# POSTECH-CVLab/NeRF-Downstream

Hardware: AMD Instinct MI355X
Metric: voxels/sec fwd+bwd Mink-ResNet14 on CO3D plenoxels (higher is better)
Workload: dtype f32

## Files before the change

### include/mink_hip.h

```cpp
#ifndef MINK_HIP_H
#define MINK_HIP_H

#include <stddef.h>
#include <stdint.h>

#ifdef __cplusplus
extern "C" {
#endif

#define MINK_OK 0
#define MINK_EINVAL (-1)
#define MINK_ELAUNCH (-2)

#define MINK_STATUS_RANGE 1u
#define MINK_STATUS_UNSORTED 2u
#define MINK_STATUS_NOT_ASCENDING 4u

const char *mink_last_error(void);
int mink_abi_version(void);


int64_t mink_table_capacity(int64_t n);

int64_t mink_unique_workspace_bytes(int64_t n);
// ... 171 lines not shown
int mink_bn_stats_from_sums(const double *sums, const double *n_total, int32_t C, float eps, float momentum,
                            float *mean, float *invstd, float *running_mean, float *running_var,
                            void *stream);
int mink_bn_bwd_from_sums(const float *dy, const float *x, const float *y, int64_t n, int32_t C,
                          const double *sums, const double *n_total, const float *mean,
                          const float *invstd, const float *gamma, int32_t relu, float *dx,
                          float *dresidual, float *scratch2c, void *stream);

int mink_bn_relu_pool_fwd(const float *x, int32_t C, const float *mean, const float *invstd,
                          const float *gamma, const float *beta, const int32_t *nbr, int64_t n_out,
                          int32_t K, float *y, void *stream);
int mink_bn_relu_pool_bwd(const float *dy_pool, const float *x, int64_t n, int32_t C, const float *mean,
                          const float *invstd, const float *gamma, const float *beta,
                          const int32_t *in2out, float *dx, float *dgamma, float *dbeta,
                          void *workspace, int64_t workspace_bytes, void *stream);

int mink_pool_max_fwd(const float *x, int32_t C, const int32_t *nbr, int64_t n_out, int32_t K, float *y, int32_t *arg,
                      void *stream);
int mink_pool_max_bwd(const float *dy, const int32_t *arg, int32_t C, const int32_t *nbr_t, int64_t n_in, int32_t K,
                      float *dx, void *stream);

int mink_pool_local_fwd(const float *x, int32_t ldx, int32_t C, const int32_t *nbr, int64_t n_out, int32_t K, int32_t mode,
                        float *y, int32_t *cnt, void *stream);
int mink_pool_local_bwd(const float *dy, int32_t C, const int32_t *nbr_t, int64_t n_in, int32_t K, int32_t mode,
                        const int32_t *cnt, float *dx, void *stream);
int mink_pool_local_max_fwd(const float *x, int32_t ldx, int32_t C, const int32_t *nbr, int64_t n_out, int32_t K, float *y,
                            int32_t *arg, void *stream);
int mink_pool_local_max_bwd(const float *dy, const int32_t *arg, int32_t C, const int32_t *nbr_t, int64_t n_in, int32_t K,
                            float *dx, void *stream);
int64_t mink_global_pool_workspace_bytes(int64_t n, int32_t C, int32_t B);
// ... 136 lines not shown
  int64_t ws_bytes;
} MinkExec;

typedef struct {
  MinkConvLayer conv;
  MinkNormLayer norm;
  const int32_t *nbr_pool;
  const int32_t *in2out;
  int64_t n, n_pool;
  const float *x;
  float *y;
  float *out;
  const float *g_out;
  void *xb;
  int32_t xb_ready;
} MinkStem;

typedef struct {
  MinkConvLayer conv1, conv2, down;
  MinkNormLayer norm1, norm2, normd;
  int64_t n_in, n_out;
  const float *x;
  float *y1, *h1, *y2, *yd, *sd, *out;
  const float *g_out;
  float *g_x;
  float *g_tmp;
} MinkBasicBlock;

int64_t mink_block_workspace_bytes(int64_t n_in, int64_t n_out, int32_t cin, int32_t cout);
int64_t mink_block_grad_scratch_floats(int64_t n_in, int64_t n_out, int32_t cin, int32_t cout, int32_t has_down);
// ... 94 lines not shown
```

### nerf_downstream_amd/_lib.py

```python
import ctypes
import os
import subprocess

_HERE = os.path.dirname(os.path.abspath(__file__))
LIB_PATH = os.environ.get("MINK_HIP_LIB") or os.path.join(_HERE, "libmink_hip.so")
CSRC = os.path.join(_HERE, "csrc")

_i32, _i64, _f32, _p = ctypes.c_int32, ctypes.c_int64, ctypes.c_float, ctypes.c_void_p


class KernelMapDesc(ctypes.Structure):

    _fields_ = [("in_table_keys", _p), ("in_table_vals", _p), ("in_cap", _i64), ("out_coords", _p), ("n_out", _i64),
                ("n_in", _i64), ("nbr", _p), ("nbr_t", _p), ("K", _i32), ("offsets", _i32 * 81),
                ("in_coords", _p), ("in_ts", _i32), ("blk_build", _i32), ("blk_table", _p), ("blk_base", _p), ("blk_slot", _p),
                ("blk_rowids", _p), ("blk_counter", _p), ("blk_cap", _i64)]


class ConvLayer(ctypes.Structure):

    _fields_ = [("w", _p), ("dw", _p), ("nbr", _p), ("nbr_t", _p), ("perm", _p), ("n_perm", _i64), ("K", _i32), ("cin", _i32),
                ("cout", _i32), ("stride", _i32)]


class NormLayer(ctypes.Structure):

    _fields_ = [("gamma", _p), ("beta", _p), ("running_mean", _p), ("running_var", _p), ("dgamma", _p), ("dbeta", _p),
                ("mean", _p), ("invstd", _p), ("momentum", _f32), ("eps", _f32)]


class Exec(ctypes.Structure):

    _fields_ = [("compute", _p), ("branch", _p), ("wgrad", _p), ("ws_compute", _p), ("ws_branch", _p), ("ws_wgrad", _p),
                ("ws_bytes", _i64)]


class Stem(ctypes.Structure):

    _fields_ = [("conv", ConvLayer), ("norm", NormLayer), ("nbr_pool", _p), ("in2out", _p), ("n", _i64), ("n_pool", _i64),
                ("x", _p), ("y", _p), ("out", _p), ("g_out", _p), ("xb", _p), ("xb_ready", _i32)]


class BasicBlock(ctypes.Structure):

    _fields_ = [("conv1", ConvLayer), ("conv2", ConvLayer), ("down", ConvLayer), ("norm1", NormLayer), ("norm2", NormLayer),
                ("normd", NormLayer), ("n_in", _i64), ("n_out", _i64), ("x", _p), ("y1", _p), ("h1", _p), ("y2", _p),
                ("yd", _p), ("sd", _p), ("out", _p), ("g_out", _p), ("g_x", _p), ("g_tmp", _p)]


class LevelMaps(ctypes.Structure):

    _fields_ = [("n", _i64), ("nbr3", _p), ("down3", _p), ("down1", _p), ("down3_t", _p), ("perm", _p), ("n_perm", _i64)]


class Net(ctypes.Structure):
# ... 111 lines not shown
    "mink_bn_stats": (ctypes.c_int, [_p, _i64, _i32, _f32, _f32, _p, _p, _p, _p, _p, _i64, _p]),
    "mink_bn_apply": (ctypes.c_int, [_p, _i64, _i32, _p, _p, _p, _p, _p, _i32, _p, _p]),
    "mink_bn_fwd": (ctypes.c_int, [_p, _i64, _i32, _f32, _f32, _p, _p, _p, _i32, _p, _p, _p, _p, _p, _p, _i64, _p]),
    "mink_bn_bwd": (ctypes.c_int, [_p, _p, _p, _i64, _i32, _p, _p, _p, _i32, _p, _p, _p, _p, _p, _i64, _p]),
    "mink_in_workspace_bytes": (_i64, [_i64, _i32, _i32]),
    "mink_in_fwd": (ctypes.c_int, [_p, _i64, _i32, _p, _i32, _f32, _p, _p, _p, _i32, _p, _p, _p, _p, _i64, _p]),
    "mink_in_bwd": (ctypes.c_int, [_p, _p, _p, _i64, _i32, _p, _i32, _p, _p, _p, _i32, _p, _p, _p, _p, _p, _i64, _p]),
    "mink_ln_workspace_bytes": (_i64, [_i64, _i32]),
    "mink_ln_fwd": (ctypes.c_int, [_p, _i64, _i32, _f32, _p, _p, _p, _i32, _p, _p, _p, _p]),
    "mink_ln_bwd": (ctypes.c_int, [_p, _p, _p, _i64, _i32, _p, _p, _p, _i32, _p, _p, _p, _p, _p, _i64, _p]),
    "mink_bn_reduce": (ctypes.c_int, [_i32, _p, _p, _p, _i64, _i32, _p, _p, _p, _p, _i64, _p]),
    "mink_bn_stats_from_sums": (ctypes.c_int, [_p, _p, _i32, _f32, _f32, _p, _p, _p, _p, _p]),
    "mink_bn_bwd_from_sums": (ctypes.c_int, [_p, _p, _p, _i64, _i32, _p, _p, _p, _p, _p, _i32, _p, _p, _p, _p]),
    "mink_bn_relu_pool_fwd": (ctypes.c_int, [_p, _i32, _p, _p, _p, _p, _p, _i64, _i32, _p, _p]),
    "mink_bn_relu_pool_bwd": (ctypes.c_int, [_p, _p, _i64, _i32, _p, _p, _p, _p, _p, _p, _p, _p, _p, _i64, _p]),
    "mink_eltwise": (ctypes.c_int, [_p, _p, _i64, _i32, _p, _p]),
    "mink_sgd_step": (ctypes.c_int, [_p, _p, _p, _i64, _f32, _f32, _f32, _i32, _p]),
    "mink_activation": (ctypes.c_int, [_p, _p, _p, _i32, _i64, _i32, _f32, _p, _p]),
    "mink_block_workspace_bytes": (_i64, [_i64, _i64, _i32, _i32]),
    "mink_block_grad_scratch_floats": (_i64, [_i64, _i64, _i32, _i32, _i32]),
    "mink_class_partition_batch": (ctypes.c_int, [_i32, _p, _p]),
    "mink_rows_to_bf16": (ctypes.c_int, [_p, _i64, _i32, _i32, _p, _p]),
    "mink_stem_conv_bf16s_supported": (ctypes.c_int, [_i64, _i64, _i32, _i32, _i32]),
    "mink_stem_conv_bf16s_stats_rows": (_i32, []),
    "mink_stem_conv_bf16s": (ctypes.c_int, [_p, _i64, _p, _i32, _p, _i64, _i32, _p, _i32, _p, _i32, _p]),
    "mink_bn_relu_pool_fwd_b16": (ctypes.c_int, [_p, _i32, _p, _p, _p, _p, _p, _i64, _i32, _p, _p]),
    "mink_bn_relu_pool_bwd_b16": (ctypes.c_int, [_p, _p, _i64, _i32, _p, _p, _p, _p, _p, _p, _p, _p, _i64, _p]),
    "mink_conv_wgrad_bn_relu_pool_b16": (
        ctypes.c_int,
        [_p, _i64, _i32, _p, _i32, _p, _i64, _p, _p, _p, _p, _p, _p, _p, _p, _i64, _i32, _p, _p, _i64, _p],
# ... 49 lines not shown
        if not os.path.exists(LIB_PATH):
            raise MinkHipError(
                f"{LIB_PATH} not found: the HIP backend is mandatory (no CPU fallback). "
                "Build it with `python -c 'import __graft_entry__ as g; g.build()'` or `make -C nerf_downstream_amd/csrc`."
            )
        import torch

        L = ctypes.CDLL(LIB_PATH)
        for name, (res, args) in SIGNATURES.items():
            fn = getattr(L, name)
            fn.restype, fn.argtypes = res, args
        if os.environ.get("MINK_BN_FOLD"):
            L.mink_bn_set_fold(int(os.environ["MINK_BN_FOLD"]))
        if os.environ.get("MINK_BN_SMALL"):
            L.mink_bn_set_small(int(os.environ["MINK_BN_SMALL"]))
        if os.environ.get("MINK_CONV_PIPELINE"):
            L.mink_conv_set_pipeline(int(os.environ["MINK_CONV_PIPELINE"]))
        _lib = L
    return _lib


def check(rc):
    if rc != 0:
        raise MinkHipError(f"libmink_hip: {lib().mink_last_error().decode()} (code {rc})")
```

### nerf_downstream_amd/csrc/elementwise.hip

```cpp
#include <algorithm>

#include "common.h"

namespace mink {

constexpr int EB = 256;
static bool g_bn_small = true;
static bool g_bn_fold_force = false;
static int g_bn_fold = 0;
constexpr int kRedBlocks = 2048;

__device__ __forceinline__ float4 ld4(const float *p) { return *reinterpret_cast<const float4 *>(p); }
__device__ __forceinline__ void st4(float *p, float4 v) { *reinterpret_cast<float4 *>(p) = v; }
template <bool B16>
__device__ __forceinline__ float4 ldx4(const float *p, int64_t i) {
  if constexpr (!B16) return *reinterpret_cast<const float4 *>(p + i);
  const uint2 u = *reinterpret_cast<const uint2 *>(reinterpret_cast<const unsigned short *>(p) + i);
  return make_float4(__uint_as_float(u.x << 16), __uint_as_float(u.x & 0xFFFF0000u), __uint_as_float(u.y << 16),
                     __uint_as_float(u.y & 0xFFFF0000u));
}

__device__ __forceinline__ void bn_running_update(float *running_mean, float *running_var, int c, float momentum, float m, double var, int64_t n) {
#pragma clang fp contract(off)
  const double unbiased = n > 1 ? var * (double)n / (double)(n - 1) : var;
// ... 670 lines not shown
    }
  }
}

template <bool BWD>
__global__ __launch_bounds__(EB) void activation_kernel(const float *__restrict__ x, const float *__restrict__ gy,
                                                        const float *__restrict__ slope, int C, int64_t count, int kind,
                                                        float alpha, float *__restrict__ out) {
  for (int64_t i = (int64_t)blockIdx.x * EB + threadIdx.x; i < count; i += (int64_t)gridDim.x * EB) {
    const float a = slope ? slope[C > 1 ? (int)(i % C) : 0] : alpha;
    const float v = act_eval<BWD>(kind, x[i], a);
    out[i] = BWD ? gy[i] * v : v;
  }
}

template <bool B16>
__global__ __launch_bounds__(EB) void bn_relu_pool_fwd_kernel(const float *__restrict__ x, int C4,
                                                              const float *__restrict__ mean,
                                                              const float *__restrict__ invstd,
                                                              const float *__restrict__ gamma,
                                                              const float *__restrict__ beta,
                                                              const int *__restrict__ nbr, int64_t n_out, int K,
                                                              float *__restrict__ y) {
  const int64_t idx = (int64_t)blockIdx.x * EB + threadIdx.x;
  if (idx >= n_out * C4) return;
  const int64_t o = idx / C4;
  const int c = (int)(idx - o * C4) * 4;
  const float4 mu = ld4(mean + c), is = ld4(invstd + c), g = ld4(gamma + c), b = ld4(beta + c);
  const float4 sc = make_float4(is.x * g.x, is.y * g.y, is.z * g.z, is.w * g.w);
  const float4 sh = make_float4(b.x - mu.x * sc.x, b.y - mu.y * sc.y, b.z - mu.z * sc.z, b.w - mu.w * sc.w);
  float4 s = make_float4(0, 0, 0, 0);
  auto add = [&](const float4 &v) {
    s.x += fmaxf((v.x - mu.x) * is.x * g.x + b.x, 0.f), s.y += fmaxf((v.y - mu.y) * is.y * g.y + b.y, 0.f);
    s.z += fmaxf((v.z - mu.z) * is.z * g.z + b.z, 0.f), s.w += fmaxf((v.w - mu.w) * is.w * g.w + b.w, 0.f);
  };
  if (K == 8) {
    int ch[8];
#pragma unroll
    for (int k = 0; k < 8; ++k) ch[k] = nbr[o * 8 + k];
    float4 v[8];
#pragma unroll
    for (int k = 0; k < 8; ++k) v[k] = ldx4<B16>(x, (int64_t)max(ch[k], 0) * (4 * C4) + c);
#pragma unroll
    for (int k = 0; k < 8; ++k)
      if (ch[k] >= 0) add(v[k]);
  } else {
    for (int k = 0; k < K; ++k) {
      const int i = nbr[o * K + k];
      if (i >= 0) add(ldx4<B16>(x, (int64_t)i * (4 * C4) + c));
    }
  }
  (void)sh;
  st4(y + o * (int64_t)(4 * C4) + c, s);
}

__global__ __launch_bounds__(EB) void bn_relu_pool_bwd_kernel(const float *__restrict__ dyp,
                                                              const float *__restrict__ x,
                                                              const int *__restrict__ in2out, int64_t n, int C4,
                                                              float inv_n, const float *__restrict__ mean,
                                                              const float *__restrict__ invstd,
                                                              const float *__restrict__ gamma,
                                                              const float *__restrict__ beta,
                                                              const float *__restrict__ dgamma,
                                                              const float *__restrict__ dbeta,
                                                              float *__restrict__ dx) {
  for (int64_t i4 = (int64_t)blockIdx.x * EB + threadIdx.x; i4 < n * C4; i4 += (int64_t)gridDim.x * EB) {
    const int64_t row = i4 / C4;
    const int c = (int)(i4 - row * C4) * 4;
// ... 463 lines not shown
  REQ_C4(C, "bn_bwd_from_sums");
  MINK_REQUIRE(n >= 1 && dy && x && sums && n_total && mean && invstd && gamma && dx && scratch2c,
               "bn_bwd_from_sums: bad arguments");
  MINK_REQUIRE(!relu || y, "bn_bwd_from_sums: fused ReLU needs the forward output");
  hipStream_t st = (hipStream_t)stream;
  bn_bwd_sums_to_float_kernel<<<dim3((unsigned)cdiv(C, 64)), 64, 0, st>>>(sums, n_total, C, scratch2c, scratch2c + C);
  MINK_CHECK_LAUNCH();
  const int64_t n4 = n * (C >> 2);
  bn_bwd_apply_kernel<<<dim3(ew_grid(n4)), EB, 0, st>>>(dy, x, relu ? y : nullptr, n4, C >> 2, 1.f, mean, invstd, gamma,
                                                       scratch2c + C, scratch2c, dx, dresidual);
  MINK_CHECK_LAUNCH();
  return MINK_OK;
}

static int bn_relu_pool_fwd_impl(const float *x, bool b16, int32_t C, const float *mean, const float *invstd, const float *gamma,
                                 const float *beta, const int32_t *nbr, int64_t n_out, int32_t K, float *y, void *stream) {
  REQ_C4(C, "bn_relu_pool_fwd");
  MINK_REQUIRE(n_out >= 0 && K >= 1, "bn_relu_pool_fwd: bad shape");
  if (n_out == 0) return MINK_OK;
  MINK_REQUIRE(x && mean && invstd && gamma && beta && nbr && y, "bn_relu_pool_fwd: NULL pointer");
  REQ_A16(x, "bn_relu_pool_fwd");
  REQ_A16(y, "bn_relu_pool_fwd");
  const dim3 grid((unsigned)cdiv(n_out * (C >> 2), EB));
  if (b16) bn_relu_pool_fwd_kernel<true><<<grid, EB, 0, (hipStream_t)stream>>>(x, C >> 2, mean, invstd, gamma, beta, nbr, n_out, K, y);
  else bn_relu_pool_fwd_kernel<false><<<grid, EB, 0, (hipStream_t)stream>>>(x, C >> 2, mean, invstd, gamma, beta, nbr, n_out, K, y);
  MINK_CHECK_LAUNCH();
  return MINK_OK;
}

int mink_bn_relu_pool_fwd(const float *x, int32_t C, const float *mean, const float *invstd, const float *gamma,
                          const float *beta, const int32_t *nbr, int64_t n_out, int32_t K, float *y, void *stream) {
  return bn_relu_pool_fwd_impl(x, false, C, mean, invstd, gamma, beta, nbr, n_out, K, y, stream);
}

int mink_bn_relu_pool_fwd_b16(const void *xb, int32_t C, const float *mean, const float *invstd, const float *gamma,
                              const float *beta, const int32_t *nbr, int64_t n_out, int32_t K, float *y, void *stream) {
  return bn_relu_pool_fwd_impl((const float *)xb, true, C, mean, invstd, gamma, beta, nbr, n_out, K, y, stream);
}

static int bn_relu_pool_bwd_impl(const float *dy_pool, const float *x, bool b16, int64_t n, int32_t C, const float *mean,
// ... 191 lines not shown
```

### nerf_downstream_amd/csrc/trunk.hip

```cpp
#include <algorithm>
#include <vector>

#include "common.h"

namespace mink {
namespace {

struct Scratch {
  char *base;
  int64_t bytes, off = 0;
  Scratch(void *p, int64_t n) : base((char *)p), bytes(n) {}
  void *take(int64_t n) {
    n = align_up(n > 0 ? n : 1, 256);
    if (!base || off + n > bytes) return nullptr;
    void *p = base + off;
    off += n;
    return p;
  }
};

constexpr int kEvents = 8;
hipEvent_t g_ev[kEvents];
bool g_ev_ready = false;

// ... 190 lines not shown
    const int rows = mink_stem_conv_bf16s_stats_rows();
    double *partial = (double *)ws.take((int64_t)rows * 2 * c.cout * sizeof(double));
    MINK_REQUIRE(partial, "stem_forward: scratch too small");
    if (!s->xb_ready) TRY(mink_rows_to_bf16(s->x, s->n, c.cin, c.cin, s->xb, st));
    TRY(mink_stem_conv_bf16s(s->xb, s->n, c.w, c.cin, c.nbr, s->n, c.K, s->y, c.cout, partial, rows, st));
    TRY(mink_bn_stats_from_partials(partial, rows, s->n, c.cout, s->norm.eps, s->norm.running_mean ? s->norm.momentum : 0.f, s->norm.mean,
                                    s->norm.invstd, s->norm.running_mean, s->norm.running_var, st));
    return mink_bn_relu_pool_fwd_b16(s->y, c.cout, s->norm.mean, s->norm.invstd, s->norm.gamma, s->norm.beta, s->nbr_pool, s->n_pool, 8,
                                     s->out, st);
  }
  ConvOut co;
  TRY(conv_stats(s->conv, s->norm, s->x, s->n, s->n, s->y, ex->ws_compute, ex->ws_bytes, st, co));
  if (co.rows > 0)
    TRY(mink_bn_stats_from_partials(co.partial, co.rows, s->n, s->conv.cout, s->norm.eps, s->norm.running_mean ? s->norm.momentum : 0.f,
                                    s->norm.mean, s->norm.invstd, s->norm.running_mean, s->norm.running_var, st));
  return mink_bn_relu_pool_fwd(s->y, s->conv.cout, s->norm.mean, s->norm.invstd, s->norm.gamma, s->norm.beta, s->nbr_pool,
                               s->n_pool, 8, s->out, st);
}

int mink_stem_backward(const MinkStem *s, const MinkExec *ex) {
  MINK_REQUIRE(s && ex, "stem_backward: NULL descriptor");
  TRY(check_conv(s->conv, "stem_backward", true));
  TRY(check_norm(s->norm, "stem_backward", true));
  MINK_REQUIRE(s->x && s->y && s->g_out && s->in2out && s->n >= 1 && s->n_pool >= 1, "stem_backward: bad arguments");
  hipStream_t st = (hipStream_t)ex->compute;
  Scratch ws(ex->ws_compute, ex->ws_bytes);
  void *bn_ws = ws.take(mink_bn_workspace_bytes(s->n, s->conv.cout));
  const int64_t need = mink_conv_wgrad_workspace_bytes(s->n, s->conv.K, s->conv.cin, s->conv.cout);
  void *slabs = need > 0 ? ws.take(need) : nullptr;
  MINK_REQUIRE(bn_ws && (need == 0 || slabs), "stem_backward: scratch too small");
  if (s->xb) {
    TRY(mink_bn_relu_pool_bwd_b16(s->g_out, s->y, s->n, s->conv.cout, s->norm.mean, s->norm.invstd, s->norm.gamma, s->norm.beta, s->in2out,
                                  s->norm.dgamma, s->norm.dbeta, bn_ws, mink_bn_workspace_bytes(s->n, s->conv.cout), st));
    return mink_conv_wgrad_bn_relu_pool_b16(s->xb, s->n, s->conv.cin, s->y, s->conv.cout, s->g_out, s->n_pool, s->in2out, s->norm.mean,
                                            s->norm.invstd, s->norm.gamma, s->norm.beta, s->norm.dgamma, s->norm.dbeta, s->conv.nbr,
                                            s->n, s->conv.K, s->conv.dw, slabs, need, st);
  }
  TRY(mink_bn_relu_pool_bwd(s->g_out, s->y, s->n, s->conv.cout, s->norm.mean, s->norm.invstd, s->norm.gamma, s->norm.beta,
                            s->in2out, nullptr, s->norm.dgamma, s->norm.dbeta, bn_ws, mink_bn_workspace_bytes(s->n, s->conv.cout), st));
  return mink_conv_wgrad_bn_relu_pool(s->x, s->n, s->conv.cin, s->conv.cin, s->y, s->conv.cout, s->g_out, s->n_pool, s->in2out,
                                      s->norm.mean, s->norm.invstd, s->norm.gamma, s->norm.beta, s->norm.dgamma,
                                      s->norm.dbeta, s->conv.nbr, s->n, s->conv.K, s->conv.dw, slabs, need, st);
}

int mink_block_forward(const MinkBasicBlock *b, const MinkExec *ex) {
  MINK_REQUIRE(b && ex, "block_forward: NULL descriptor");
  TRY(check_conv(b->conv1, "block_forward conv1", false));
  TRY(check_conv(b->conv2, "block_forward conv2", false));
  TRY(check_norm(b->norm1, "block_forward norm1", false));
  TRY(check_norm(b->norm2, "block_forward norm2", false));
  const bool down = b->down.w != nullptr;
  const int C = b->conv1.cout;
  MINK_REQUIRE(b->x && b->y1 && b->h1 && b->y2 && b->out && b->n_in >= 1 && b->n_out >= 1 && b->conv2.cin == C &&
                   b->conv2.cout == C,
// ... 172 lines not shown
  b.norm1.mean = st, b.norm1.invstd = st + C, b.norm2.mean = st + 2 * C, b.norm2.invstd = st + 3 * C;
  b.normd.mean = st + 4 * C, b.normd.invstd = st + 5 * C;
  b.conv2.nbr = lo.nbr3, b.conv2.nbr_t = nullptr, b.conv2.perm = nullptr, b.conv2.n_perm = 0;
  if (b.conv1.stride == 2) {
    b.conv1.nbr = lo.down3, b.conv1.nbr_t = lo.down3_t, b.conv1.perm = lo.perm, b.conv1.n_perm = lo.perm ? lo.n_perm : 0;
    MINK_REQUIRE(sh.down && lo.down1, "net: a strided block needs its shortcut convolution and the k=1 table");
    b.down.nbr = lo.down1, b.down.nbr_t = nullptr, b.down.perm = nullptr, b.down.n_perm = 0;
  } else {
    MINK_REQUIRE(!sh.down, "net: a stride-1 block with a shortcut convolution is not sequenced here");
    b.conv1.nbr = lo.nbr3, b.conv1.nbr_t = nullptr, b.conv1.perm = nullptr, b.conv1.n_perm = 0;
  }
  MINK_REQUIRE(b.conv1.nbr && b.conv2.nbr, "net: missing neighbour table at level %d", sh.level_out);
  return MINK_OK;
}

}

extern "C" {

int mink_set_block_done_hook(MinkBlockDoneHook hook) {
  g_block_done_hook = hook;
  return MINK_OK;
}

int mink_set_stage_hook(MinkStageHook hook) {
  g_stage_hook = hook;
  return MINK_OK;
}

int mink_event_create(void **event_out) {
// ... 14 lines not shown
  MINK_HIP(hipStreamWaitEvent((hipStream_t)stream, (hipEvent_t)event, 0));
  return MINK_OK;
}

int mink_net_sizes(const MinkNet *net, const MinkLevelMaps *levels, int32_t n_levels, int64_t *act_floats, int64_t *grad_floats,
                   int64_t *ws_bytes) {
  MINK_REQUIRE(net && levels && n_levels >= 1 && net->n_blocks >= 1 && net->blocks, "net_sizes: bad arguments");
  int64_t act = 0, grad = 0, ws = 0;
  int level = 0;
  for (int i = 0; i < net->n_blocks; ++i) {
    BlockShape sh;
    TRY(block_shape(net, levels, n_levels, i, level, sh));
    act += sh.act + sh.stats, grad += sh.gtmp + sh.gx;
    ws = std::max(ws, mink_block_workspace_bytes(sh.n_in, sh.n_out, net->blocks[i].conv1.cin, net->blocks[i].conv1.cout));
  }
  if (act_floats) *act_floats = act;
  if (grad_floats) *grad_floats = grad;
  if (ws_bytes) *ws_bytes = ws;
  return MINK_OK;
}

int mink_net_forward(MinkNet *net, const MinkLevelMaps *levels, int32_t n_levels, float *arena, int64_t arena_floats,
                     const MinkExec *ex) {
  MINK_REQUIRE(net && levels && arena && ex && net->blocks && net->n_blocks >= 1, "net_forward: bad arguments");
  if (g_stage_hook) g_stage_hook(-1, 0);
  if (net->with_stem) TRY(mink_stem_forward(&net->stem, ex));
  MINK_REQUIRE(net->stem.out && net->stem.n_pool == levels[0].n, "net_forward: the stem output must be level 0 (%lld rows, %lld given)",
               (long long)net->stem.n_pool, (long long)levels[0].n);
  const float *x = net->stem.out;
  int level = 0;
  int64_t off = 0;
  for (int i = 0; i < net->n_blocks; ++i) {
    BlockShape sh;
    TRY(block_shape(net, levels, n_levels, i, level, sh));
    MINK_REQUIRE(off + sh.act + sh.stats <= arena_floats, "net_forward: activation arena of %lld floats is too small (mink_net_sizes)",
                 (long long)arena_floats);
    MinkBasicBlock &b = net->blocks[i];
    TRY(bind_block(b, sh, levels, arena + off, x));
    b.g_out = nullptr, b.g_x = nullptr, b.g_tmp = nullptr;
    if (g_stage_hook) g_stage_hook(i, 0);
    TRY(mink_block_forward(&b, ex));
// ... 7 lines not shown

int mink_net_backward(MinkNet *net, const MinkLevelMaps *levels, int32_t n_levels, float *arena, int64_t arena_floats,
                      const float *g_out, float *grad_arena, int64_t grad_floats, const MinkExec *ex, void *const *done_events) {
  MINK_REQUIRE(net && levels && arena && g_out && grad_arena && ex && net->blocks && net->n_blocks >= 1, "net_backward: bad arguments");
  TRY(ensure_events());
  std::vector<BlockShape> shapes(net->n_blocks);
  std::vector<int64_t> offs(net->n_blocks);
  int level = 0;
  int64_t off = 0, goff_total = 0;
  for (int i = 0; i < net->n_blocks; ++i) {
    TRY(block_shape(net, levels, n_levels, i, level, shapes[i]));
    offs[i] = off;
    off += shapes[i].act + shapes[i].stats;
    goff_total += shapes[i].gtmp + shapes[i].gx;
  }
  MINK_REQUIRE(off <= arena_floats && goff_total <= grad_floats, "net_backward: arena too small (mink_net_sizes)");
  hipStream_t st = (hipStream_t)ex->compute, wst = (hipStream_t)ex->wgrad;
  const float *g = g_out;
  int64_t goff = 0;
  PendingGrad pending;
  for (int i = net->n_blocks - 1; i >= 0; --i) {
    const BlockShape &sh = shapes[i];
    MinkBasicBlock &b = net->blocks[i];
    const float *x = i == 0 ? net->stem.out : arena + offs[i - 1] + 3 * shapes[i - 1].n_out * net->blocks[i - 1].conv1.cout;
    TRY(bind_block(b, sh, levels, arena + offs[i], x));
    b.g_out = g, b.g_tmp = grad_arena + goff, b.g_x = grad_arena + goff + sh.gtmp;
    if (g_stage_hook) g_stage_hook(i, 1);
    const bool may_defer = i > 0 && shapes[i - 1].level_out == sh.level_out && net->blocks[i - 1].conv1.cout == b.conv1.cin;
    PendingGrad next;
    TRY(block_backward_impl(&b, ex, &pending, may_defer ? &next : nullptr));
    pending = next;
    const bool want_event = done_events && done_events[i];
    if (want_event || g_block_done_hook) {
      if (wst != st) TRY(order_after(wst, st, 7));
      if ((hipStream_t)ex->branch != st && (hipStream_t)ex->branch != wst) TRY(order_after(wst, (hipStream_t)ex->branch, 4));
      if (want_event) MINK_HIP(hipEventRecord((hipEvent_t)done_events[i], wst));
      if (g_block_done_hook) g_block_done_hook(i);
    }
    g = b.g_x;
    goff += sh.gtmp + sh.gx;
  }
  if (g_stage_hook) g_stage_hook(-1, 1);
  if (net->with_stem) {
    net->stem.g_out = g;
    TRY(mink_stem_backward(&net->stem, ex));
  }
  net->g_stem_out = g;
  return MINK_OK;
}

}
```

### nerf_downstream_amd/minkowski/functional.py

```python
import ctypes
import os

import torch

from .._lib import check, lib


def _stream():
    return torch._C._cuda_getCurrentRawStream(torch.cuda.current_device())


def _f32c(t):
    assert t.is_cuda, "the HIP backend has no CPU path"
    return t.contiguous() if t.dtype == torch.float32 else t.float().contiguous()


def _ptr(t):
    return None if t is None else t.data_ptr()


def _bytes(nbytes, device):
    return torch.empty(max(int(nbytes), 256), dtype=torch.uint8, device=device)


# ... 761 lines not shown
        )
        dbeta, dgamma = sums[:C].float(), sums[C:].float()
        dist.all_reduce(sums, group=ctx.group)
        gx = torch.empty_like(x)
        gres = torch.empty_like(x) if ctx.has_res else None
        tmp = torch.empty(2 * C, dtype=torch.float32, device=dev)
        check(
            L.mink_bn_bwd_from_sums(
                gy.data_ptr(), x.data_ptr(), _ptr(y), n, C, sums.data_ptr(), n_total.data_ptr(), mean.data_ptr(),
                invstd.data_ptr(), gamma.data_ptr(), int(ctx.relu), gx.data_ptr(), _ptr(gres), tmp.data_ptr(), _stream(),
            )
        )
        return gx, dgamma, dbeta, None, None, None, None, gres, None, None


class BNReLUSumPoolFunction(torch.autograd.Function):

    @staticmethod
    def forward(ctx, x, gamma, beta, running_mean, running_var, training, momentum, eps, nbr, in2out, partial=None):
        L = lib()
        x = _f32c(x)
        n, C = x.shape
        dev = x.device
        if training:
            mean, invstd = _bn_statistics(L, x, n, C, eps, momentum, running_mean, running_var, partial)
        else:
            mean = running_mean.float()
            invstd = torch.rsqrt(running_var.float() + eps)
        n_out, K = nbr.shape
        y = torch.empty(n_out, C, dtype=torch.float32, device=dev)
        check(
            L.mink_bn_relu_pool_fwd(
                x.data_ptr(), C, mean.data_ptr(), invstd.data_ptr(), gamma.data_ptr(), beta.data_ptr(), nbr.data_ptr(),
                n_out, K, y.data_ptr(), _stream(),
            )
        )
        ctx.save_for_backward(x, mean, invstd, gamma, beta)
        ctx.in2out, ctx.training = in2out, training
        return y

    @staticmethod
    def backward(ctx, gy):
        if not ctx.training:
            raise NotImplementedError("fused bn+relu+pool backward needs batch statistics (training mode)")
        L = lib()
        x, mean, invstd, gamma, beta = ctx.saved_tensors
        gy = _f32c(gy)
        n, C = x.shape
        gx = torch.empty_like(x)
        dgamma = torch.empty(C, dtype=torch.float32, device=x.device)
        dbeta = torch.empty(C, dtype=torch.float32, device=x.device)
        ws = _scratch(L.mink_bn_workspace_bytes(n, C), x.device, "bn")
        check(
            L.mink_bn_relu_pool_bwd(
                gy.data_ptr(), x.data_ptr(), n, C, mean.data_ptr(), invstd.data_ptr(), gamma.data_ptr(), beta.data_ptr(),
                ctx.in2out.data_ptr(), gx.data_ptr(), dgamma.data_ptr(), dbeta.data_ptr(), ws.data_ptr(), ws.numel(), _stream(),
            )
        )
        return gx, dgamma, dbeta, None, None, None, None, None, None, None, None


class ConvBNReLUSumPoolFunction(torch.autograd.Function):

    @staticmethod
    def forward(ctx, x, kernel, gamma, beta, running_mean, running_var, momentum, eps, nbr, nbr_pool, in2out):
        L = lib()
        x, w = _f32c(x), _f32c(kernel)
        cin = x.shape[1]
        ctx.cin = cin
        if cin % 4:
            pad = 4 - cin % 4
            x = torch.nn.functional.pad(x, (0, pad))
            w = torch.nn.functional.pad(w, (0, 0, 0, pad))
        C = w.shape[-1]
        y, partial = gather_gemm(x, w, nbr, C, stats=True)
        n = y.shape[0]
        mean, invstd = _bn_statistics(L, y, n, C, eps, momentum, running_mean, running_var, partial)
        n_pool, K = nbr_pool.shape
        out = torch.empty(n_pool, C, dtype=torch.float32, device=x.device)
        check(
            L.mink_bn_relu_pool_fwd(
                y.data_ptr(), C, mean.data_ptr(), invstd.data_ptr(), gamma.data_ptr(), beta.data_ptr(), nbr_pool.data_ptr(),
                n_pool, K, out.data_ptr(), _stream(),
            )
        )
        ctx.save_for_backward(x, w, y, mean, invstd, gamma, beta)
        ctx.nbr, ctx.in2out = nbr, in2out
        ctx.kernel = kernel
        return out

    @staticmethod
    def backward(ctx, gy):
        L = lib()
        x, w, y, mean, invstd, gamma, beta = ctx.saved_tensors
        gy = _f32c(gy)
        n, C = y.shape
        dev = y.device
        need = ctx.needs_input_grad
        pv = _sink_views(gamma, beta) if need[2] and need[3] else None
        kv = _sink_views(ctx.kernel) if need[1] and w.shape[1] == ctx.cin else None
        if pv is not None:
            dgamma, dbeta = pv
        else:
            dgamma = torch.empty(C, dtype=torch.float32, device=dev)
            dbeta = torch.empty(C, dtype=torch.float32, device=dev)
        gw = kv[0] if kv is not None else None
        ws = _scratch(L.mink_bn_workspace_bytes(n, C), dev, "bn")
        check(
            L.mink_bn_relu_pool_bwd(
                gy.data_ptr(), y.data_ptr(), n, C, mean.data_ptr(), invstd.data_ptr(), gamma.data_ptr(), beta.data_ptr(),
                ctx.in2out.data_ptr(), None, dgamma.data_ptr(), dbeta.data_ptr(), ws.data_ptr(), ws.numel(), _stream(),
            )
        )
        nbr = ctx.nbr
        K = nbr.shape[1]
        if gw is None:
            gw = torch.empty(w.shape, dtype=torch.float32, device=dev)
        wws = _scratch(L.mink_conv_wgrad_workspace_bytes(n, K, x.shape[1], C), dev, "wgrad")
        note_table(nbr)
        check(
            L.mink_conv_wgrad_bn_relu_pool(
                x.data_ptr(), x.shape[0], x.stride(0), x.shape[1], y.data_ptr(), C, gy.data_ptr(), gy.shape[0],
                ctx.in2out.data_ptr(), mean.data_ptr(), invstd.data_ptr(), gamma.data_ptr(), beta.data_ptr(),
                dgamma.data_ptr(), dbeta.data_ptr(), nbr.data_ptr(), n, K, gw.data_ptr(), wws.data_ptr(), wws.numel(), _stream(),
            )
        )
        if _GRAD_SINK is not None and hasattr(_GRAD_SINK, "flush"):
            _GRAD_SINK.flush()
# ... 537 lines not shown
```

Before: 241.3 million.

## Compute stem BN-ReLU-pool gradient reductions from pooled-resolution byproducts

The forward BN+ReLU+sum-pool kernel now also records, per pooled row and channel, the count of children that passed ReLU (uint8) and the sum of their normalized values. The backward dgamma/dbeta reduction then reads these pooled-resolution tensors instead of re-reading the full-resolution pre-pool activations with in2out indirection. This shrinks the reduction's memory traffic by roughly the pooling factor, at the cost of extra forward writes and extra arena memory. It is on by default and also changes the Python autograd path.

```diff
diff --git a/include/mink_hip.h b/include/mink_hip.h
--- a/include/mink_hip.h
+++ b/include/mink_hip.h
@@ -209,6 +209,17 @@
                           const float *invstd, const float *gamma, const float *beta,
                           const int32_t *in2out, float *dx, float *dgamma, float *dbeta,
                           void *workspace, int64_t workspace_bytes, void *stream);
+int mink_bn_relu_pool_fwd_stats(const float *x, int32_t C, const float *mean, const float *invstd, const float *gamma,
+                                const float *beta, const int32_t *nbr, int64_t n_out, int32_t K, float *y, uint8_t *cnt,
+                                float *xs, void *stream);
+int mink_bn_relu_pool_bwd_pooled(const float *dy_pool, const uint8_t *cnt, const float *xs, int64_t n_pool, int32_t C,
+                                 const float *gamma, float *dgamma, float *dbeta, void *workspace, int64_t workspace_bytes,
+                                 void *stream);
+int mink_bn_relu_pool_bwd_dx(const float *dy_pool, const float *x, int64_t n, int32_t C, const float *mean, const float *invstd,
+                             const float *gamma, const float *beta, const int32_t *in2out, const float *dgamma,
+                             const float *dbeta, float *dx, void *stream);
+int32_t mink_stem_pooled_bwd(void);
+int mink_stem_set_pooled_bwd(int32_t on);
 
 int mink_pool_max_fwd(const float *x, int32_t C, const int32_t *nbr, int64_t n_out, int32_t K, float *y, int32_t *arg,
                       void *stream);
@@ -375,6 +386,8 @@
   const float *g_out;
   void *xb;
   int32_t xb_ready;
+  uint8_t *pool_cnt;
+  float *pool_xs;
 } MinkStem;
 
 typedef struct {
diff --git a/nerf_downstream_amd/_lib.py b/nerf_downstream_amd/_lib.py
--- a/nerf_downstream_amd/_lib.py
+++ b/nerf_downstream_amd/_lib.py
@@ -38,7 +38,7 @@
 class Stem(ctypes.Structure):
 
     _fields_ = [("conv", ConvLayer), ("norm", NormLayer), ("nbr_pool", _p), ("in2out", _p), ("n", _i64), ("n_pool", _i64),
-                ("x", _p), ("y", _p), ("out", _p), ("g_out", _p), ("xb", _p), ("xb_ready", _i32)]
+                ("x", _p), ("y", _p), ("out", _p), ("g_out", _p), ("xb", _p), ("xb_ready", _i32), ("pool_cnt", _p), ("pool_xs", _p)]
 
 
 class BasicBlock(ctypes.Structure):
@@ -180,6 +180,11 @@
     "mink_bn_bwd_from_sums": (ctypes.c_int, [_p, _p, _p, _i64, _i32, _p, _p, _p, _p, _p, _i32, _p, _p, _p, _p]),
     "mink_bn_relu_pool_fwd": (ctypes.c_int, [_p, _i32, _p, _p, _p, _p, _p, _i64, _i32, _p, _p]),
     "mink_bn_relu_pool_bwd": (ctypes.c_int, [_p, _p, _i64, _i32, _p, _p, _p, _p, _p, _p, _p, _p, _p, _i64, _p]),
+    "mink_bn_relu_pool_fwd_stats": (ctypes.c_int, [_p, _i32, _p, _p, _p, _p, _p, _i64, _i32, _p, _p, _p, _p]),
+    "mink_bn_relu_pool_bwd_pooled": (ctypes.c_int, [_p, _p, _p, _i64, _i32, _p, _p, _p, _p, _i64, _p]),
+    "mink_bn_relu_pool_bwd_dx": (ctypes.c_int, [_p, _p, _i64, _i32, _p, _p, _p, _p, _p, _p, _p, _p, _p]),
+    "mink_stem_pooled_bwd": (_i32, []),
+    "mink_stem_set_pooled_bwd": (ctypes.c_int, [_i32]),
     "mink_eltwise": (ctypes.c_int, [_p, _p, _i64, _i32, _p, _p]),
     "mink_sgd_step": (ctypes.c_int, [_p, _p, _p, _i64, _f32, _f32, _f32, _i32, _p]),
     "mink_activation": (ctypes.c_int, [_p, _p, _p, _i32, _i64, _i32, _f32, _p, _p]),
@@ -259,6 +264,8 @@
             L.mink_bn_set_fold(int(os.environ["MINK_BN_FOLD"]))
         if os.environ.get("MINK_BN_SMALL"):
             L.mink_bn_set_small(int(os.environ["MINK_BN_SMALL"]))
+        if os.environ.get("MINK_STEM_POOLED_BWD"):
+            L.mink_stem_set_pooled_bwd(int(os.environ["MINK_STEM_POOLED_BWD"]))
         if os.environ.get("MINK_CONV_PIPELINE"):
             L.mink_conv_set_pipeline(int(os.environ["MINK_CONV_PIPELINE"]))
         _lib = L
diff --git a/nerf_downstream_amd/csrc/elementwise.hip b/nerf_downstream_amd/csrc/elementwise.hip
--- a/nerf_downstream_amd/csrc/elementwise.hip
+++ b/nerf_downstream_amd/csrc/elementwise.hip
@@ -8,6 +8,7 @@
 static bool g_bn_small = true;
 static bool g_bn_fold_force = false;
 static int g_bn_fold = 0;
+static bool g_pool_bwd = true;
 constexpr int kRedBlocks = 2048;
 
 __device__ __forceinline__ float4 ld4(const float *p) { return *reinterpret_cast<const float4 *>(p); }
@@ -708,14 +709,15 @@
   }
 }
 
-template <bool B16>
+template <bool B16, bool PROD = false>
 __global__ __launch_bounds__(EB) void bn_relu_pool_fwd_kernel(const float *__restrict__ x, int C4,
                                                               const float *__restrict__ mean,
                                                               const float *__restrict__ invstd,
                                                               const float *__restrict__ gamma,
                                                               const float *__restrict__ beta,
                                                               const int *__restrict__ nbr, int64_t n_out, int K,
-                                                              float *__restrict__ y) {
+                                                              float *__restrict__ y, unsigned char *__restrict__ cnt = nullptr,
+                                                              float *__restrict__ xs = nullptr) {
   const int64_t idx = (int64_t)blockIdx.x * EB + threadIdx.x;
   if (idx >= n_out * C4) return;
   const int64_t o = idx / C4;
@@ -724,9 +726,19 @@
   const float4 sc = make_float4(is.x * g.x, is.y * g.y, is.z * g.z, is.w * g.w);
   const float4 sh = make_float4(b.x - mu.x * sc.x, b.y - mu.y * sc.y, b.z - mu.z * sc.z, b.w - mu.w * sc.w);
   float4 s = make_float4(0, 0, 0, 0);
+  float4 hs = make_float4(0, 0, 0, 0);
+  unsigned pass = 0;
   auto add = [&](const float4 &v) {
-    s.x += fmaxf((v.x - mu.x) * is.x * g.x + b.x, 0.f), s.y += fmaxf((v.y - mu.y) * is.y * g.y + b.y, 0.f);
-    s.z += fmaxf((v.z - mu.z) * is.z * g.z + b.z, 0.f), s.w += fmaxf((v.w - mu.w) * is.w * g.w + b.w, 0.f);
+    const float4 t = make_float4((v.x - mu.x) * is.x * g.x + b.x, (v.y - mu.y) * is.y * g.y + b.y, (v.z - mu.z) * is.z * g.z + b.z,
+                                 (v.w - mu.w) * is.w * g.w + b.w);
+    s.x += fmaxf(t.x, 0.f), s.y += fmaxf(t.y, 0.f);
+    s.z += fmaxf(t.z, 0.f), s.w += fmaxf(t.w, 0.f);
+    if constexpr (PROD) {
+      if (t.x > 0.f) hs.x += (v.x - mu.x) * is.x, pass += 1u;
+      if (t.y > 0.f) hs.y += (v.y - mu.y) * is.y, pass += 1u << 8;
+      if (t.z > 0.f) hs.z += (v.z - mu.z) * is.z, pass += 1u << 16;
+      if (t.w > 0.f) hs.w += (v.w - mu.w) * is.w, pass += 1u << 24;
+    }
   };
   if (K == 8) {
     int ch[8];
@@ -746,6 +758,55 @@
   }
   (void)sh;
   st4(y + o * (int64_t)(4 * C4) + c, s);
+  if constexpr (PROD) {
+    st4(xs + o * (int64_t)(4 * C4) + c, hs);
+    *reinterpret_cast<unsigned *>(cnt + o * (int64_t)(4 * C4) + c) = pass;
+  }
+}
+
+constexpr int kPoolRows = 8;
+constexpr int kPoolRedBlocks = 1024;
+__global__ __launch_bounds__(EB) void bn_relu_pool_bwd_pooled_kernel(const float *__restrict__ g, const unsigned char *__restrict__ cnt,
+                                                                     const float *__restrict__ xs, int64_t n, int C,
+                                                                     double *__restrict__ partial) {
+  extern __shared__ double s_red[];
+  const int tpr = C >> 2, rlanes = EB / tpr;
+  const int c4 = threadIdx.x % tpr, rl = threadIdx.x / tpr;
+  if (rl < rlanes) {
+    double a0 = 0, a1 = 0, a2 = 0, a3 = 0, b0 = 0, b1 = 0, b2 = 0, b3 = 0;
+    const int64_t stride = (int64_t)gridDim.x * rlanes;
+    for (int64_t row = (int64_t)blockIdx.x * rlanes + rl; row < n; row += kPoolRows * stride) {
+      float4 gs[kPoolRows], hs[kPoolRows];
+      unsigned cs[kPoolRows];
+#pragma unroll
+      for (int u = 0; u < kPoolRows; ++u) {
+        const int64_t r = row + u * stride < n ? row + u * stride : row;
+        const int64_t off = r * C + 4 * c4;
+        gs[u] = ld4(g + off), hs[u] = ld4(xs + off);
+        cs[u] = *reinterpret_cast<const unsigned *>(cnt + off);
+      }
+#pragma unroll
+      for (int u = 0; u < kPoolRows; ++u) {
+        if (row + u * stride < n) {
+          const float4 gv = gs[u], hv = hs[u];
+          const unsigned cv = cs[u];
+          a0 += (double)gv.x * (double)(cv & 255u), a1 += (double)gv.y * (double)((cv >> 8) & 255u);
+          a2 += (double)gv.z * (double)((cv >> 16) & 255u), a3 += (double)gv.w * (double)(cv >> 24);
+          b0 += (double)gv.x * (double)hv.x, b1 += (double)gv.y * (double)hv.y;
+          b2 += (double)gv.z * (double)hv.z, b3 += (double)gv.w * (double)hv.w;
+        }
+      }
+    }
+    double *d = s_red + ((int64_t)rl * 2) * C + 4 * c4;
+    d[0] = a0, d[1] = a1, d[2] = a2, d[3] = a3;
+    d[C + 0] = b0, d[C + 1] = b1, d[C + 2] = b2, d[C + 3] = b3;
+  }
+  __syncthreads();
+  for (int e = threadIdx.x; e < 2 * C; e += EB) {
+    double t = 0.0;
+    for (int r = 0; r < rlanes; ++r) t += s_red[(int64_t)r * 2 * C + e];
+    partial[(int64_t)blockIdx.x * 2 * C + e] = t;
+  }
 }
 
 __global__ __launch_bounds__(EB) void bn_relu_pool_bwd_kernel(const float *__restrict__ dyp,
@@ -1239,16 +1300,74 @@
 }
 
 static int bn_relu_pool_fwd_impl(const float *x, bool b16, int32_t C, const float *mean, const float *invstd, const float *gamma,
-                                 const float *beta, const int32_t *nbr, int64_t n_out, int32_t K, float *y, void *stream) {
+                                 const float *beta, const int32_t *nbr, int64_t n_out, int32_t K, float *y, void *stream,
+                                 uint8_t *cnt = nullptr, float *xs = nullptr) {
   REQ_C4(C, "bn_relu_pool_fwd");
   MINK_REQUIRE(n_out >= 0 && K >= 1, "bn_relu_pool_fwd: bad shape");
+  MINK_REQUIRE((cnt == nullptr) == (xs == nullptr), "bn_relu_pool_fwd_stats: cnt and xs come in pairs");
+  MINK_REQUIRE(!cnt || (K <= 255 && !b16), "bn_relu_pool_fwd_stats: at most 255 children per pooled row, fp32 storage");
   if (n_out == 0) return MINK_OK;
   MINK_REQUIRE(x && mean && invstd && gamma && beta && nbr && y, "bn_relu_pool_fwd: NULL pointer");
   REQ_A16(x, "bn_relu_pool_fwd");
   REQ_A16(y, "bn_relu_pool_fwd");
+  REQ_A16(cnt, "bn_relu_pool_fwd_stats");
+  REQ_A16(xs, "bn_relu_pool_fwd_stats");
   const dim3 grid((unsigned)cdiv(n_out * (C >> 2), EB));
-  if (b16) bn_relu_pool_fwd_kernel<true><<<grid, EB, 0, (hipStream_t)stream>>>(x, C >> 2, mean, invstd, gamma, beta, nbr, n_out, K, y);
+  if (cnt) bn_relu_pool_fwd_kernel<false, true><<<grid, EB, 0, (hipStream_t)stream>>>(x, C >> 2, mean, invstd, gamma, beta, nbr, n_out, K, y, cnt, xs);
+  else if (b16) bn_relu_pool_fwd_kernel<true><<<grid, EB, 0, (hipStream_t)stream>>>(x, C >> 2, mean, invstd, gamma, beta, nbr, n_out, K, y);
   else bn_relu_pool_fwd_kernel<false><<<grid, EB, 0, (hipStream_t)stream>>>(x, C >> 2, mean, invstd, gamma, beta, nbr, n_out, K, y);
+  MINK_CHECK_LAUNCH();
+  return MINK_OK;
+}
+
+int mink_bn_relu_pool_fwd_stats(const float *x, int32_t C, const float *mean, const float *invstd, const float *gamma, const float *beta,
+                                const int32_t *nbr, int64_t n_out, int32_t K, float *y, uint8_t *cnt, float *xs, void *stream) {
+  return bn_relu_pool_fwd_impl(x, false, C, mean, invstd, gamma, beta, nbr, n_out, K, y, stream, cnt, xs);
+}
+
+int32_t mink_stem_pooled_bwd(void) { return g_pool_bwd ? 1 : 0; }
+
+int mink_stem_set_pooled_bwd(int32_t on) {
+  const int old = g_pool_bwd ? 1 : 0;
+  g_pool_bwd = on != 0;
+  return old;
+}
+
+int mink_bn_relu_pool_bwd_pooled(const float *dy_pool, const uint8_t *cnt, const float *xs, int64_t n_pool, int32_t C, const float *gamma,
+                                 float *dgamma, float *dbeta, void *workspace, int64_t workspace_bytes, void *stream) {
+  REQ_C4(C, "bn_relu_pool_bwd_pooled");
+  MINK_REQUIRE(workspace_bytes >= mink_bn_workspace_bytes(n_pool, C), "bn_relu_pool_bwd_pooled: workspace of %lld bytes, %lld needed",
+               (long long)workspace_bytes, (long long)(mink_bn_workspace_bytes(n_pool, C)));
+  MINK_REQUIRE(n_pool >= 1 && dy_pool && cnt && xs && gamma && dgamma && dbeta && workspace, "bn_relu_pool_bwd_pooled: bad arguments");
+  REQ_A16(dy_pool, "bn_relu_pool_bwd_pooled");
+  REQ_A16(cnt, "bn_relu_pool_bwd_pooled");
+  REQ_A16(xs, "bn_relu_pool_bwd_pooled");
+  hipStream_t st = (hipStream_t)stream;
+  const int tpr = C >> 2;
+  MINK_REQUIRE(tpr <= EB, "bn_relu_pool_bwd_pooled: too many channels");
+  const int rlanes = EB / tpr;
+  int64_t nblk = cdiv(n_pool, (int64_t)rlanes * kPoolRows);
+  if (nblk > kPoolRedBlocks) nblk = kPoolRedBlocks;
+  static_assert(kPoolRedBlocks <= kRedBlocks, "the partials must fit mink_bn_workspace_bytes");
+  const size_t shm = (size_t)rlanes * 2 * C * sizeof(double);
+  bn_relu_pool_bwd_pooled_kernel<<<dim3((unsigned)nblk), EB, shm, st>>>(dy_pool, cnt, xs, n_pool, C, (double *)workspace);
+  MINK_CHECK_LAUNCH();
+  launch_bwd_finalize((const double *)workspace, (int)nblk, C, gamma, dgamma, dbeta, st);
+  MINK_CHECK_LAUNCH();
+  return MINK_OK;
+}
+
+int mink_bn_relu_pool_bwd_dx(const float *dy_pool, const float *x, int64_t n, int32_t C, const float *mean, const float *invstd,
+                             const float *gamma, const float *beta, const int32_t *in2out, const float *dgamma, const float *dbeta,
+                             float *dx, void *stream) {
+  REQ_C4(C, "bn_relu_pool_bwd_dx");
+  MINK_REQUIRE(n >= 1 && dy_pool && x && mean && invstd && gamma && beta && in2out && dgamma && dbeta && dx, "bn_relu_pool_bwd_dx: bad arguments");
+  REQ_A16(dy_pool, "bn_relu_pool_bwd_dx");
+  REQ_A16(x, "bn_relu_pool_bwd_dx");
+  REQ_A16(dx, "bn_relu_pool_bwd_dx");
+  const int64_t n4 = n * (C >> 2);
+  bn_relu_pool_bwd_kernel<<<dim3(ew_grid(n4)), EB, 0, (hipStream_t)stream>>>(dy_pool, x, in2out, n, C >> 2, 1.f / (float)n, mean, invstd, gamma,
+                                                                          beta, dgamma, dbeta, dx);
   MINK_CHECK_LAUNCH();
   return MINK_OK;
 }
diff --git a/nerf_downstream_amd/csrc/trunk.hip b/nerf_downstream_amd/csrc/trunk.hip
--- a/nerf_downstream_amd/csrc/trunk.hip
+++ b/nerf_downstream_amd/csrc/trunk.hip
@@ -228,8 +228,9 @@
   if (co.rows > 0)
     TRY(mink_bn_stats_from_partials(co.partial, co.rows, s->n, s->conv.cout, s->norm.eps, s->norm.running_mean ? s->norm.momentum : 0.f,
                                     s->norm.mean, s->norm.invstd, s->norm.running_mean, s->norm.running_var, st));
-  return mink_bn_relu_pool_fwd(s->y, s->conv.cout, s->norm.mean, s->norm.invstd, s->norm.gamma, s->norm.beta, s->nbr_pool,
-                               s->n_pool, 8, s->out, st);
+  MINK_REQUIRE((s->pool_cnt == nullptr) == (s->pool_xs == nullptr), "stem_forward: pool_cnt and pool_xs come in pairs");
+  return mink_bn_relu_pool_fwd_stats(s->y, s->conv.cout, s->norm.mean, s->norm.invstd, s->norm.gamma, s->norm.beta, s->nbr_pool,
+                                     s->n_pool, 8, s->out, s->pool_cnt, s->pool_xs, st);
 }
 
 int mink_stem_backward(const MinkStem *s, const MinkExec *ex) {
@@ -250,8 +251,13 @@
                                             s->norm.invstd, s->norm.gamma, s->norm.beta, s->norm.dgamma, s->norm.dbeta, s->conv.nbr,
                                             s->n, s->conv.K, s->conv.dw, slabs, need, st);
   }
-  TRY(mink_bn_relu_pool_bwd(s->g_out, s->y, s->n, s->conv.cout, s->norm.mean, s->norm.invstd, s->norm.gamma, s->norm.beta,
-                            s->in2out, nullptr, s->norm.dgamma, s->norm.dbeta, bn_ws, mink_bn_workspace_bytes(s->n, s->conv.cout), st));
+  MINK_REQUIRE((s->pool_cnt == nullptr) == (s->pool_xs == nullptr), "stem_backward: pool_cnt and pool_xs come in pairs");
+  if (s->pool_cnt)
+    TRY(mink_bn_relu_pool_bwd_pooled(s->g_out, s->pool_cnt, s->pool_xs, s->n_pool, s->conv.cout, s->norm.gamma, s->norm.dgamma,
+                                     s->norm.dbeta, bn_ws, mink_bn_workspace_bytes(s->n, s->conv.cout), st));
+  else
+    TRY(mink_bn_relu_pool_bwd(s->g_out, s->y, s->n, s->conv.cout, s->norm.mean, s->norm.invstd, s->norm.gamma, s->norm.beta,
+                              s->in2out, nullptr, s->norm.dgamma, s->norm.dbeta, bn_ws, mink_bn_workspace_bytes(s->n, s->conv.cout), st));
   return mink_conv_wgrad_bn_relu_pool(s->x, s->n, s->conv.cin, s->conv.cin, s->y, s->conv.cout, s->g_out, s->n_pool, s->in2out,
                                       s->norm.mean, s->norm.invstd, s->norm.gamma, s->norm.beta, s->norm.dgamma,
                                       s->norm.dbeta, s->conv.nbr, s->n, s->conv.K, s->conv.dw, slabs, need, st);
@@ -454,6 +460,21 @@
   return MINK_OK;
 }
 
+int64_t stem_pool_floats(const MinkNet *net, const MinkLevelMaps *levels, int64_t *cnt_off = nullptr) {
+  if (!net->with_stem || net->stem.conv.cout <= 0) return 0;
+  const int64_t elems = levels[0].n * net->stem.conv.cout;
+  const int64_t xs = align_up(elems, kNetAlign);
+  if (cnt_off) *cnt_off = xs;
+  return xs + align_up((elems + 3) / 4, kNetAlign);
+}
+
+void bind_stem_pool(MinkNet *net, const MinkLevelMaps *levels, float *tail) {
+  int64_t cnt_off = 0;
+  const bool on = stem_pool_floats(net, levels, &cnt_off) > 0 && !net->stem.xb && mink_stem_pooled_bwd();
+  net->stem.pool_xs = on ? tail : nullptr;
+  net->stem.pool_cnt = on ? reinterpret_cast<uint8_t *>(tail + cnt_off) : nullptr;
+}
+
 }
 
 extern "C" {
@@ -498,6 +519,7 @@
     act += sh.act + sh.stats, grad += sh.gtmp + sh.gx;
     ws = std::max(ws, mink_block_workspace_bytes(sh.n_in, sh.n_out, net->blocks[i].conv1.cin, net->blocks[i].conv1.cout));
   }
+  act += stem_pool_floats(net, levels);
   if (act_floats) *act_floats = act;
   if (grad_floats) *grad_floats = grad;
   if (ws_bytes) *ws_bytes = ws;
@@ -508,7 +530,19 @@
                      const MinkExec *ex) {
   MINK_REQUIRE(net && levels && arena && ex && net->blocks && net->n_blocks >= 1, "net_forward: bad arguments");
   if (g_stage_hook) g_stage_hook(-1, 0);
-  if (net->with_stem) TRY(mink_stem_forward(&net->stem, ex));
+  if (net->with_stem) {
+    int64_t blocks_floats = 0;
+    int lv = 0;
+    for (int i = 0; i < net->n_blocks; ++i) {
+      BlockShape sh;
+      TRY(block_shape(net, levels, n_levels, i, lv, sh));
+      blocks_floats += sh.act + sh.stats;
+    }
+    MINK_REQUIRE(blocks_floats + stem_pool_floats(net, levels) <= arena_floats,
+                 "net_forward: activation arena of %lld floats is too small (mink_net_sizes)", (long long)arena_floats);
+    bind_stem_pool(net, levels, arena + blocks_floats);
+    TRY(mink_stem_forward(&net->stem, ex));
+  }
   MINK_REQUIRE(net->stem.out && net->stem.n_pool == levels[0].n, "net_forward: the stem output must be level 0 (%lld rows, %lld given)",
                (long long)net->stem.n_pool, (long long)levels[0].n);
   const float *x = net->stem.out;
@@ -546,7 +580,7 @@
     off += shapes[i].act + shapes[i].stats;
     goff_total += shapes[i].gtmp + shapes[i].gx;
   }
-  MINK_REQUIRE(off <= arena_floats && goff_total <= grad_floats, "net_backward: arena too small (mink_net_sizes)");
+  MINK_REQUIRE(off + stem_pool_floats(net, levels) <= arena_floats && goff_total <= grad_floats, "net_backward: arena too small (mink_net_sizes)");
   hipStream_t st = (hipStream_t)ex->compute, wst = (hipStream_t)ex->wgrad;
   const float *g = g_out;
   int64_t goff = 0;
@@ -575,6 +609,7 @@
   if (g_stage_hook) g_stage_hook(-1, 1);
   if (net->with_stem) {
     net->stem.g_out = g;
+    bind_stem_pool(net, levels, arena + off);
     TRY(mink_stem_backward(&net->stem, ex));
   }
   net->g_stem_out = g;
diff --git a/nerf_downstream_amd/minkowski/functional.py b/nerf_downstream_amd/minkowski/functional.py
--- a/nerf_downstream_amd/minkowski/functional.py
+++ b/nerf_downstream_amd/minkowski/functional.py
@@ -799,6 +799,12 @@
         return gx, dgamma, dbeta, None, None, None, None, gres, None, None
 
 
+def _pool_byproducts(L, n_out, C, K, dev):
+    if not L.mink_stem_pooled_bwd() or K > 255 or n_out == 0:
+        return None, None
+    return torch.empty(n_out, C, dtype=torch.uint8, device=dev), torch.empty(n_out, C, dtype=torch.float32, device=dev)
+
+
 class BNReLUSumPoolFunction(torch.autograd.Function):
 
     @staticmethod
@@ -814,14 +820,15 @@
             invstd = torch.rsqrt(running_var.float() + eps)
         n_out, K = nbr.shape
         y = torch.empty(n_out, C, dtype=torch.float32, device=dev)
-        check(
-            L.mink_bn_relu_pool_fwd(
+        cnt, xs = _pool_byproducts(L, n_out, C, K, dev) if (training and any(ctx.needs_input_grad[:3])) else (None, None)
+        check(
+            L.mink_bn_relu_pool_fwd_stats(
                 x.data_ptr(), C, mean.data_ptr(), invstd.data_ptr(), gamma.data_ptr(), beta.data_ptr(), nbr.data_ptr(),
-                n_out, K, y.data_ptr(), _stream(),
+                n_out, K, y.data_ptr(), _ptr(cnt), _ptr(xs), _stream(),
             )
         )
         ctx.save_for_backward(x, mean, invstd, gamma, beta)
-        ctx.in2out, ctx.training = in2out, training
+        ctx.in2out, ctx.training, ctx.pooled = in2out, training, (cnt, xs)
         return y
 
     @staticmethod
@@ -836,6 +843,21 @@
         dgamma = torch.empty(C, dtype=torch.float32, device=x.device)
         dbeta = torch.empty(C, dtype=torch.float32, device=x.device)
         ws = _scratch(L.mink_bn_workspace_bytes(n, C), x.device, "bn")
+        cnt, xs = ctx.pooled
+        if cnt is not None:
+            check(
+                L.mink_bn_relu_pool_bwd_pooled(
+                    gy.data_ptr(), cnt.data_ptr(), xs.data_ptr(), gy.shape[0], C, gamma.data_ptr(), dgamma.data_ptr(), dbeta.data_ptr(),
+                    ws.data_ptr(), ws.numel(), _stream(),
+                )
+            )
+            check(
+                L.mink_bn_relu_pool_bwd_dx(
+                    gy.data_ptr(), x.data_ptr(), n, C, mean.data_ptr(), invstd.data_ptr(), gamma.data_ptr(), beta.data_ptr(),
+                    ctx.in2out.data_ptr(), dgamma.data_ptr(), dbeta.data_ptr(), gx.data_ptr(), _stream(),
+                )
+            )
+            return gx, dgamma, dbeta, None, None, None, None, None, None, None, None
         check(
             L.mink_bn_relu_pool_bwd(
                 gy.data_ptr(), x.data_ptr(), n, C, mean.data_ptr(), invstd.data_ptr(), gamma.data_ptr(), beta.data_ptr(),
@@ -863,14 +885,15 @@
         mean, invstd = _bn_statistics(L, y, n, C, eps, momentum, running_mean, running_var, partial)
         n_pool, K = nbr_pool.shape
         out = torch.empty(n_pool, C, dtype=torch.float32, device=x.device)
-        check(
-            L.mink_bn_relu_pool_fwd(
+        cnt, xs = _pool_byproducts(L, n_pool, C, K, x.device)
+        check(
+            L.mink_bn_relu_pool_fwd_stats(
                 y.data_ptr(), C, mean.data_ptr(), invstd.data_ptr(), gamma.data_ptr(), beta.data_ptr(), nbr_pool.data_ptr(),
-                n_pool, K, out.data_ptr(), _stream(),
+                n_pool, K, out.data_ptr(), _ptr(cnt), _ptr(xs), _stream(),
             )
         )
         ctx.save_for_backward(x, w, y, mean, invstd, gamma, beta)
-        ctx.nbr, ctx.in2out = nbr, in2out
+        ctx.nbr, ctx.in2out, ctx.pooled = nbr, in2out, (cnt, xs)
         ctx.kernel = kernel
         return out
 
@@ -891,12 +914,21 @@
             dbeta = torch.empty(C, dtype=torch.float32, device=dev)
         gw = kv[0] if kv is not None else None
         ws = _scratch(L.mink_bn_workspace_bytes(n, C), dev, "bn")
-        check(
-            L.mink_bn_relu_pool_bwd(
-                gy.data_ptr(), y.data_ptr(), n, C, mean.data_ptr(), invstd.data_ptr(), gamma.data_ptr(), beta.data_ptr(),
-                ctx.in2out.data_ptr(), None, dgamma.data_ptr(), dbeta.data_ptr(), ws.data_ptr(), ws.numel(), _stream(),
-            )
-        )
+        cnt, xs = ctx.pooled
+        if cnt is not None:
+            check(
+                L.mink_bn_relu_pool_bwd_pooled(
+                    gy.data_ptr(), cnt.data_ptr(), xs.data_ptr(), gy.shape[0], C, gamma.data_ptr(), dgamma.data_ptr(), dbeta.data_ptr(),
+                    ws.data_ptr(), ws.numel(), _stream(),
+                )
+            )
+        else:
+            check(
+                L.mink_bn_relu_pool_bwd(
+                    gy.data_ptr(), y.data_ptr(), n, C, mean.data_ptr(), invstd.data_ptr(), gamma.data_ptr(), beta.data_ptr(),
+                    ctx.in2out.data_ptr(), None, dgamma.data_ptr(), dbeta.data_ptr(), ws.data_ptr(), ws.numel(), _stream(),
+                )
+            )
         nbr = ctx.nbr
         K = nbr.shape[1]
         if gw is None:
```

Result: no change. 243.0 million (median of 5 runs) (+0.7%).
